# CompVis/stable-diffusion

Measured on NVIDIA B200. Metric: images_per_sec_sdv1_512x512_plms50_cfg7.5, higher is better.
Workload: dtype fp16

## Files before the change

### stable-diffusion_b200/csrc/attention_tc.cu

```cuda
#include "../../include/sdb200.h"
#include "host.h"
#include "ptx.cuh"

#include <stdlib.h>

namespace sdb {

constexpr int AQ = 128;
constexpr int AKV = 64;
template <int DPAD>
struct AttnCfg {
  static constexpr int ST = DPAD <= 128 ? 3 : 2;
  static constexpr int SMEM = AQ * DPAD * 2 + ST * (2 * AKV * DPAD * 2) + 2 * AQ * AKV * 2 + 1024;
};

struct AttnArgs {
  int nq, nkv, d, heads;
  int ldo;
  long long o_batch_stride;
  __half* out;
  float scale_log2;
  int causal;
};

__device__ __forceinline__ float fast_exp2(float x) {
  float y;
  asm("ex2.approx.ftz.f32 %0, %1;" : "=f"(y) : "f"(x));
  return y;
}

template <int DPAD>
__global__ void __launch_bounds__(192)
    attention_tc_kernel(const __grid_constant__ CUtensorMap tmQ, const __grid_constant__ CUtensorMap tmK,
                        const __grid_constant__ CUtensorMap tmV, const AttnArgs p) {
  constexpr int PANELS = DPAD / 64;
  constexpr int Q_BYTES = AQ * DPAD * 2;
  constexpr int K_BYTES = AKV * DPAD * 2;
  constexpr int V_BYTES = DPAD * AKV * 2;
  constexpr int P_BYTES = AQ * AKV * 2;
  constexpr int TMEM_COLS = (128 + DPAD) <= 256 ? 256 : 512;
  constexpr int ST = AttnCfg<DPAD>::ST;
  constexpr uint32_t O_COL = 128;

  extern __shared__ uint8_t smem_raw[];
  uint8_t* smem = smem_raw + ((1024u - (smem_u32(smem_raw) & 1023u)) & 1023u);
  uint8_t* q_s = smem;
  uint8_t* k_s = q_s + Q_BYTES;
  uint8_t* v_s = k_s + ST * K_BYTES;
  uint8_t* p_s = v_s + ST * V_BYTES;

  __shared__ uint64_t q_full, k_full[ST], v_full[ST], kv_empty[ST], s_full[2], p_full[2], pv_done[2];
  __shared__ uint32_t tmem_base_smem;

  const int warp = threadIdx.x >> 5;
  const int lane = threadIdx.x & 31;
  pdl_launch_dependents();
  const int q0 = blockIdx.x * AQ;
  const int head = blockIdx.y;
  const int b = blockIdx.z;
  int nkv_eff = p.nkv;
  if (p.causal) nkv_eff = min(p.nkv, q0 + AQ);
  const int n_iter = (nkv_eff + AKV - 1) / AKV;

  if (warp == 0 && lane == 0) {
    tma_prefetch_desc(&tmQ);
    tma_prefetch_desc(&tmK);
    tma_prefetch_desc(&tmV);
    mbar_init(&q_full, 1);
    for (int i = 0; i < ST; ++i) {
      mbar_init(&k_full[i], 1);
      mbar_init(&v_full[i], 1);
      mbar_init(&kv_empty[i], 1);
    }
    for (int i = 0; i < 2; ++i) {
      mbar_init(&s_full[i], 1);
      mbar_init(&p_full[i], 128);
      mbar_init(&pv_done[i], 1);
    }
    fence_barrier_init();
  }
  if (warp == 1) {
    tmem_alloc(&tmem_base_smem, TMEM_COLS);
    tmem_relinquish();
  }
  tc_fence_before();
  __syncthreads();
  tc_fence_after();
  const uint32_t tmem = tmem_base_smem;

  pdl_wait();
  if (warp == 0) {
    if (elect_one()) {
      mbar_arrive_expect_tx(&q_full, Q_BYTES);
      for (int pn = 0; pn < PANELS; ++pn)
        tma_load_3d(q_s + pn * (AQ * 128), &tmQ, &q_full, head * DPAD + pn * 64, q0, b);
      for (int j = 0; j < n_iter; ++j) {
        int s = j % ST;
        uint32_t ph = (j / ST) & 1;
        mbar_wait(&kv_empty[s], ph ^ 1);
        mbar_arrive_expect_tx(&k_full[s], K_BYTES);
        for (int pn = 0; pn < PANELS; ++pn)
          tma_load_3d(k_s + s * K_BYTES + pn * (AKV * 128), &tmK, &k_full[s], head * DPAD + pn * 64, j * AKV, b);
        mbar_arrive_expect_tx(&v_full[s], V_BYTES);
        tma_load_3d(v_s + s * V_BYTES, &tmV, &v_full[s], j * AKV, head * DPAD, b);
      }
    }
  } else if (warp == 1) {
    if (elect_one()) {
      constexpr uint32_t idesc_s = umma_idesc_f16(AQ, AKV);
      const int ksteps = (p.d + 15) >> 4;
      const uint32_t idesc_o = umma_idesc_f16(AQ, ksteps * 16);
      const uint32_t q_addr = smem_u32(q_s);
      auto issue_s = [&](int j) {
        const int s = j & 1;
        const int ks = j % ST;
        mbar_wait(&k_full[ks], (j / ST) & 1);
        tc_fence_after();
        const uint32_t k_addr = smem_u32(k_s + ks * K_BYTES);
#pragma unroll
        for (int kk = 0; kk < DPAD / 16; ++kk) {
          if (kk >= ksteps) break;
          uint64_t da = umma_desc_k128(q_addr + (kk >> 2) * (AQ * 128) + (kk & 3) * 32);
          uint64_t db = umma_desc_k128(k_addr + (kk >> 2) * (AKV * 128) + (kk & 3) * 32);
          umma_f16(tmem + s * AKV, da, db, idesc_s, kk > 0 ? 1u : 0u);
        }
        umma_commit(&s_full[s]);
      };
      mbar_wait(&q_full, 0);
      if (n_iter > 0) issue_s(0);
      for (int j = 0; j < n_iter; ++j) {
        int s = j & 1;
        uint32_t ph = (j >> 1) & 1;
        if (j + 1 < n_iter) issue_s(j + 1);
        const int ks = j % ST;
        mbar_wait(&p_full[s], ph);
        mbar_wait(&v_full[ks], (j / ST) & 1);
        tc_fence_after();
        const uint32_t p_addr = smem_u32(p_s + s * P_BYTES);
        const uint32_t v_addr = smem_u32(v_s + ks * V_BYTES);
#pragma unroll
        for (int kk = 0; kk < AKV / 16; ++kk) {
          uint64_t da = umma_desc_k128(p_addr + kk * 32);
          uint64_t db = umma_desc_k128(v_addr + kk * 32);
          umma_f16(tmem + O_COL, da, db, idesc_o, (j > 0 || kk > 0) ? 1u : 0u);
        }
        umma_commit(&kv_empty[ks]);
        umma_commit(&pv_done[s]);
      }
    }
  } else {
    const int lg = warp & 3;
    const int r = lg * 32 + lane;
    const int qi = q0 + r;
    const uint32_t lane_addr = static_cast<uint32_t>(lg * 32) << 16;
    float m_used = -INFINITY;
    float l = 0.f;
    for (int j = 0; j < n_iter; ++j) {
      const int s = j & 1;
      mbar_wait(&s_full[s], (j >> 1) & 1);
      tc_fence_after();
      float t[AKV];
      {
        uint32_t r0[32], r1[32];
        tmem_ld32(tmem + lane_addr + s * AKV, r0);
        tmem_ld32(tmem + lane_addr + s * AKV + 32, r1);
        tmem_ld_wait();
#pragma unroll
        for (int c = 0; c < 32; ++c) {
          t[c] = __uint_as_float(r0[c]);
          t[32 + c] = __uint_as_float(r1[c]);
        }
      }
      const int kv0 = j * AKV;
      if ((kv0 + AKV > p.nkv) || (p.causal && kv0 + AKV - 1 > q0)) {
#pragma unroll
        for (int c = 0; c < AKV; ++c) {
          int kv = kv0 + c;
          if ((kv >= p.nkv) || (p.causal && kv > qi)) t[c] = -INFINITY;
        }
      }
      float mx[8];
#pragma unroll
      for (int i = 0; i < 8; ++i) mx[i] = t[i];
#pragma unroll
      for (int c = 8; c < AKV; ++c) mx[c & 7] = fmaxf(mx[c & 7], t[c]);
      const float m_raw = fmaxf(fmaxf(fmaxf(mx[0], mx[1]), fmaxf(mx[2], mx[3])), fmaxf(fmaxf(mx[4], mx[5]), fmaxf(mx[6], mx[7])));
      const float m_blk = m_raw * p.scale_log2;
      if (j == 0) {
        m_used = m_blk;
      } else {
        float m_new = fmaxf(m_used, m_blk);
        bool need = m_new > m_used + 8.0f;
        if (__any_sync(0xffffffffu, need)) {
          mbar_wait(&pv_done[(j - 1) & 1], ((j - 1) >> 1) & 1);
          tc_fence_after();
          float alpha = need ? exp2f(m_used - m_new) : 1.0f;
#pragma unroll 1
          for (int c = 0; c < DPAD / 32; ++c) {
            uint32_t o[32];
            tmem_ld32(tmem + lane_addr + O_COL + c * 32, o);
            tmem_ld_wait();
#pragma unroll
            for (int i = 0; i < 32; ++i) o[i] = __float_as_uint(__uint_as_float(o[i]) * alpha);
            tmem_st32(tmem + lane_addr + O_COL + c * 32, o);
          }
          tmem_st_wait();
          l *= alpha;
          if (need) m_used = m_new;
        }
      }
      float sm[8] = {0.f, 0.f, 0.f, 0.f, 0.f, 0.f, 0.f, 0.f};
      const float neg_m = -m_used;
      if (j >= 2) mbar_wait(&pv_done[s], ((j - 2) >> 1) & 1);
#pragma unroll
      for (int c = 0; c < AKV; ++c) {
        t[c] = fast_exp2(fmaf(t[c], p.scale_log2, neg_m));
        sm[c & 7] += t[c];
      }
      l += ((sm[0] + sm[1]) + (sm[2] + sm[3])) + ((sm[4] + sm[5]) + (sm[6] + sm[7]));
      uint8_t* prow = p_s + s * P_BYTES + r * 128;
#pragma unroll
      for (int c16 = 0; c16 < 8; ++c16) {
        __half2 h0 = __floats2half2_rn(t[c16 * 8 + 0], t[c16 * 8 + 1]);
        __half2 h1 = __floats2half2_rn(t[c16 * 8 + 2], t[c16 * 8 + 3]);
        __half2 h2 = __floats2half2_rn(t[c16 * 8 + 4], t[c16 * 8 + 5]);
        __half2 h3 = __floats2half2_rn(t[c16 * 8 + 6], t[c16 * 8 + 7]);
        uint4 u;
        u.x = *reinterpret_cast<uint32_t*>(&h0);
        u.y = *reinterpret_cast<uint32_t*>(&h1);
        u.z = *reinterpret_cast<uint32_t*>(&h2);
        u.w = *reinterpret_cast<uint32_t*>(&h3);
        *reinterpret_cast<uint4*>(prow + ((c16 ^ (r & 7)) << 4)) = u;
      }
      fence_proxy_async();
      tc_fence_before();
      mbar_arrive(&p_full[s]);
    }
    if (n_iter > 0) {
      mbar_wait(&pv_done[(n_iter - 1) & 1], ((n_iter - 1) >> 1) & 1);
      tc_fence_after();
    }
    const float inv_l = l > 0.f ? 1.0f / l : 0.f;
    __half* orow = p.out + static_cast<size_t>(b) * p.o_batch_stride + static_cast<size_t>(qi) * p.ldo + head * p.d;
#pragma unroll 1
    for (int c = 0; c < DPAD / 32; ++c) {
      if (c * 32 >= p.d) break;
      uint32_t o[32];
      tmem_ld32(tmem + lane_addr + O_COL + c * 32, o);
      tmem_ld_wait();
      if (qi < p.nq && n_iter > 0) {
#pragma unroll
        for (int i = 0; i < 32; i += 2) {
          int col = c * 32 + i;
          if (col < p.d)
            *reinterpret_cast<__half2*>(orow + col) =
                __floats2half2_rn(__uint_as_float(o[i]) * inv_l, __uint_as_float(o[i + 1]) * inv_l);
        }
      }
    }
    tc_fence_before();
  }
  __syncthreads();
  if (warp == 1) {
    tc_fence_after();
    tmem_dealloc(tmem, TMEM_COLS);
  }
}


constexpr int SPLIT_THREADS = 64 + 256;
constexpr int SPLIT_ST = 3;
constexpr int SPLIT_SMEM = AQ * 64 * 2 + SPLIT_ST * (2 * AKV * 64 * 2) + 2 * AQ * AKV * 2 + 1024;

__global__ void __launch_bounds__(SPLIT_THREADS, 2)
    attention_split_kernel(const __grid_constant__ CUtensorMap tmQ, const __grid_constant__ CUtensorMap tmK,
                           const __grid_constant__ CUtensorMap tmV, const AttnArgs p) {
  constexpr int DPAD = 64;
  constexpr int Q_BYTES = AQ * DPAD * 2;
  constexpr int K_BYTES = AKV * DPAD * 2;
  constexpr int V_BYTES = DPAD * AKV * 2;
  constexpr int P_BYTES = AQ * AKV * 2;
  constexpr int TMEM_COLS = 256;
  constexpr int ST = SPLIT_ST;
  constexpr uint32_t O_COL = 128;

  extern __shared__ uint8_t smem_raw[];
  uint8_t* smem = smem_raw + ((1024u - (smem_u32(smem_raw) & 1023u)) & 1023u);
  uint8_t* q_s = smem;
  uint8_t* k_s = q_s + Q_BYTES;
  uint8_t* v_s = k_s + ST * K_BYTES;
  uint8_t* p_s = v_s + ST * V_BYTES;

  __shared__ uint64_t q_full, k_full[ST], v_full[ST], kv_empty[ST], s_full[2], p_full[2], pv_done[2];
  __shared__ uint32_t tmem_base_smem;
  __shared__ float m_sh[2][AQ];

  const int warp = threadIdx.x >> 5;
  const int lane = threadIdx.x & 31;
  pdl_launch_dependents();
  const int q0 = blockIdx.x * AQ;
  const int head = blockIdx.y;
  const int b = blockIdx.z;
  int nkv_eff = p.nkv;
  if (p.causal) nkv_eff = min(p.nkv, q0 + AQ);
  const int n_iter = (nkv_eff + AKV - 1) / AKV;

  if (warp == 0 && lane == 0) {
    tma_prefetch_desc(&tmQ);
    tma_prefetch_desc(&tmK);
    tma_prefetch_desc(&tmV);
    mbar_init(&q_full, 1);
    for (int i = 0; i < ST; ++i) {
      mbar_init(&k_full[i], 1);
      mbar_init(&v_full[i], 1);
      mbar_init(&kv_empty[i], 1);
    }
    for (int i = 0; i < 2; ++i) {
      mbar_init(&s_full[i], 1);
      mbar_init(&p_full[i], 256);
      mbar_init(&pv_done[i], 1);
    }
    fence_barrier_init();
  }
  if (warp == 1) {
    tmem_alloc(&tmem_base_smem, TMEM_COLS);
    tmem_relinquish();
  }
  {
    const int granules = (DPAD - p.d) * 8;
    for (int i = threadIdx.x; i < ST * granules; i += SPLIT_THREADS) {
      const int st = i / granules, g = i - st * granules;
      const uint32_t val = (g < 8) ? 0x3C003C00u : 0u;
      *reinterpret_cast<uint4*>(v_s + st * V_BYTES + p.d * 128 + g * 16) = make_uint4(val, val, val, val);
    }
    fence_proxy_async();
  }
  tc_fence_before();
  __syncthreads();
  tc_fence_after();
  const uint32_t tmem = tmem_base_smem;

  pdl_wait();
  if (warp == 0) {
    if (elect_one()) {
      const uint32_t v_load_bytes = static_cast<uint32_t>(p.d) * AKV * 2;
      mbar_arrive_expect_tx(&q_full, Q_BYTES);
      tma_load_3d(q_s, &tmQ, &q_full, head * DPAD, q0, b);
      for (int j = 0; j < n_iter; ++j) {
        int s = j % ST;
        uint32_t ph = (j / ST) & 1;
        mbar_wait(&kv_empty[s], ph ^ 1);
        mbar_arrive_expect_tx(&k_full[s], K_BYTES);
        tma_load_3d(k_s + s * K_BYTES, &tmK, &k_full[s], head * DPAD, j * AKV, b);
        mbar_arrive_expect_tx(&v_full[s], v_load_bytes);
        tma_load_3d(v_s + s * V_BYTES, &tmV, &v_full[s], j * AKV, head * DPAD, b);
      }
    }
  } else if (warp == 1) {
    if (elect_one()) {
      constexpr uint32_t idesc_s = umma_idesc_f16(AQ, AKV);
      const int ksteps = (p.d + 15) >> 4;
      const uint32_t idesc_o = umma_idesc_f16(AQ, min(DPAD, ((p.d + 16) >> 4) << 4));
      const uint32_t q_addr = smem_u32(q_s);
      auto issue_s = [&](int j) {
        const int s = j & 1;
        const int ks = j % ST;
        mbar_wait(&k_full[ks], (j / ST) & 1);
        tc_fence_after();
        const uint32_t k_addr = smem_u32(k_s + ks * K_BYTES);
#pragma unroll
        for (int kk = 0; kk < DPAD / 16; ++kk) {
          if (kk >= ksteps) break;
          uint64_t da = umma_desc_k128(q_addr + kk * 32);
          uint64_t db = umma_desc_k128(k_addr + kk * 32);
          umma_f16(tmem + s * AKV, da, db, idesc_s, kk > 0 ? 1u : 0u);
        }
        umma_commit(&s_full[s]);
      };
      mbar_wait(&q_full, 0);
      if (n_iter > 0) issue_s(0);
      for (int j = 0; j < n_iter; ++j) {
        int s = j & 1;
        uint32_t ph = (j >> 1) & 1;
        if (j + 1 < n_iter) issue_s(j + 1);
        const int ks = j % ST;
        mbar_wait(&p_full[s], ph);
        mbar_wait(&v_full[ks], (j / ST) & 1);
        tc_fence_after();
        const uint32_t p_addr = smem_u32(p_s + s * P_BYTES);
        const uint32_t v_addr = smem_u32(v_s + ks * V_BYTES);
#pragma unroll
        for (int kk = 0; kk < AKV / 16; ++kk) {
          uint64_t da = umma_desc_k128(p_addr + kk * 32);
          uint64_t db = umma_desc_k128(v_addr + kk * 32);
          umma_f16(tmem + O_COL + (kk >> 1) * DPAD, da, db, idesc_o, (j > 0 || (kk & 1)) ? 1u : 0u);
        }
        umma_commit(&kv_empty[ks]);
        umma_commit(&pv_done[s]);
      }
    }
  } else {
    const int lg = warp & 3;
    const int hf = (warp - 2) >> 2;
    const int r = lg * 32 + lane;
    const int qi = q0 + r;
    const uint32_t lane_addr = static_cast<uint32_t>(lg * 32) << 16;
    const uint32_t o_addr = tmem + lane_addr + O_COL + hf * DPAD;
    float m_used = -INFINITY;
    for (int j = 0; j < n_iter; ++j) {
      const int s = j & 1;
      mbar_wait(&s_full[s], (j >> 1) & 1);
      tc_fence_after();
      float t[32];
      {
        uint32_t r0[32];
        tmem_ld32(tmem + lane_addr + s * AKV + hf * 32, r0);
        tmem_ld_wait();
#pragma unroll
        for (int c = 0; c < 32; ++c) t[c] = __uint_as_float(r0[c]);
      }
      const int kv0 = j * AKV + hf * 32;
      if ((kv0 + 32 > p.nkv) || (p.causal && kv0 + 31 > q0)) {
#pragma unroll
        for (int c = 0; c < 32; ++c) {
          int kv = kv0 + c;
          if ((kv >= p.nkv) || (p.causal && kv > qi)) t[c] = -INFINITY;
        }
      }
      float mx[4];
#pragma unroll
      for (int i = 0; i < 4; ++i) mx[i] = fmaxf(fmaxf(t[i], t[4 + i]), t[8 + i]);
#pragma unroll
      for (int i = 0; i < 4; ++i) mx[i] = fmaxf(fmaxf(mx[i], t[12 + i]), t[16 + i]);
#pragma unroll
      for (int i = 0; i < 4; ++i) mx[i] = fmaxf(fmaxf(mx[i], t[20 + i]), t[24 + i]);
#pragma unroll
      for (int i = 0; i < 4; ++i) mx[i] = fmaxf(mx[i], t[28 + i]);
      const float m_blk = fmaxf(fmaxf(mx[0], mx[1]), fmaxf(mx[2], mx[3])) * p.scale_log2;
      {
        const float m_new = fmaxf(m_used, m_blk);
        const bool need = m_new > m_used + 8.0f;
        if (j > 0 && __any_sync(0xffffffffu, need)) {
          mbar_wait(&pv_done[(j - 1) & 1], ((j - 1) >> 1) & 1);
          tc_fence_after();
          const float alpha = need ? exp2f(m_used - m_new) : 1.0f;
#pragma unroll 1
          for (int c = 0; c < DPAD / 32; ++c) {
            uint32_t o[32];
            tmem_ld32(o_addr + c * 32, o);
            tmem_ld_wait();
#pragma unroll
            for (int i = 0; i < 32; ++i) o[i] = __float_as_uint(__uint_as_float(o[i]) * alpha);
            tmem_st32(o_addr + c * 32, o);
          }
          tmem_st_wait();
        }
        if (need) m_used = m_new;
      }
      const float neg_m = (m_used == -INFINITY) ? 0.f : -m_used;
      if (j >= 2) mbar_wait(&pv_done[s], ((j - 2) >> 1) & 1);
#pragma unroll
      for (int c = 0; c < 32; ++c) t[c] = fast_exp2(fmaf(t[c], p.scale_log2, neg_m));
      uint8_t* prow = p_s + s * P_BYTES + r * 128;
#pragma unroll
      for (int i = 0; i < 4; ++i) {
        __half2 h0 = __floats2half2_rn(t[i * 8 + 0], t[i * 8 + 1]);
        __half2 h1 = __floats2half2_rn(t[i * 8 + 2], t[i * 8 + 3]);
        __half2 h2 = __floats2half2_rn(t[i * 8 + 4], t[i * 8 + 5]);
        __half2 h3 = __floats2half2_rn(t[i * 8 + 6], t[i * 8 + 7]);
        uint4 u;
        u.x = *reinterpret_cast<uint32_t*>(&h0);
        u.y = *reinterpret_cast<uint32_t*>(&h1);
        u.z = *reinterpret_cast<uint32_t*>(&h2);
        u.w = *reinterpret_cast<uint32_t*>(&h3);
        *reinterpret_cast<uint4*>(prow + (((hf * 4 + i) ^ (r & 7)) << 4)) = u;
      }
      fence_proxy_async();
      tc_fence_before();
      mbar_arrive(&p_full[s]);
    }
    m_sh[hf][r] = m_used;
    asm volatile("bar.sync 1, 256;" ::: "memory");
    if (n_iter > 0) {
      mbar_wait(&pv_done[(n_iter - 1) & 1], ((n_iter - 1) >> 1) & 1);
      tc_fence_after();
    }
    const float mA = m_sh[0][r], mB = m_sh[1][r];
    const float m = fmaxf(mA, mB);
    const float fA = (mA == -INFINITY) ? 0.f : exp2f(mA - m);
    const float fB = (mB == -INFINITY) ? 0.f : exp2f(mB - m);
    const uint32_t oa = tmem + lane_addr + O_COL, ob = oa + DPAD;
    float inv_l = 0.f;
    uint32_t a[32], bb[32];
    if (n_iter > 0) {
      const uint32_t la = tmem_ld1(oa + p.d), lb = tmem_ld1(ob + p.d);
      tmem_ld32(oa + hf * 32, a);
      tmem_ld32(ob + hf * 32, bb);
      tmem_ld_wait();
      const float l = fA * __uint_as_float(la) + fB * __uint_as_float(lb);
      inv_l = l > 0.f ? 1.0f / l : 0.f;
    }
    if (qi < p.nq && n_iter > 0) {
      __half* orow = p.out + static_cast<size_t>(b) * p.o_batch_stride + static_cast<size_t>(qi) * p.ldo + head * p.d;
      const float ga = fA * inv_l, gb = fB * inv_l;
#pragma unroll
      for (int i = 0; i < 32; i += 2) {
        const int col = hf * 32 + i;
        if (col < p.d)
          *reinterpret_cast<__half2*>(orow + col) =
              __floats2half2_rn(__uint_as_float(a[i]) * ga + __uint_as_float(bb[i]) * gb,
                                __uint_as_float(a[i + 1]) * ga + __uint_as_float(bb[i + 1]) * gb);
      }
    }
    tc_fence_before();
  }
  __syncthreads();
  if (warp == 1) {
    tc_fence_after();
    tmem_dealloc(tmem, TMEM_COLS);
  }
}


constexpr int WIDE_D = 512;
constexpr int WIDE_DV = 256;
constexpr int WIDE_KST = 4;
constexpr int WIDE_PANELS = WIDE_D / 64;
constexpr int WIDE_SMEM = AQ * WIDE_D * 2 + WIDE_KST * (AKV * 64 * 2) + WIDE_DV * AKV * 2 + AQ * AKV * 2 + 1024;

__global__ void __launch_bounds__(192, 1)
    attention_wide_kernel(const __grid_constant__ CUtensorMap tmQ, const __grid_constant__ CUtensorMap tmK,
                          const __grid_constant__ CUtensorMap tmV, const AttnArgs p) {
  constexpr int Q_BYTES = AQ * WIDE_D * 2;
  constexpr int KP_BYTES = AKV * 64 * 2;
  constexpr int V_BYTES = WIDE_DV * AKV * 2;
  constexpr int TMEM_COLS = 512;
  constexpr uint32_t O_COL = 128;

  extern __shared__ uint8_t smem_raw[];
  uint8_t* smem = smem_raw + ((1024u - (smem_u32(smem_raw) & 1023u)) & 1023u);
  uint8_t* q_s = smem;
  uint8_t* k_s = q_s + Q_BYTES;
  uint8_t* v_s = k_s + WIDE_KST * KP_BYTES;
  uint8_t* p_s = v_s + V_BYTES;

  __shared__ uint64_t q_full, k_full[WIDE_KST], k_empty[WIDE_KST], v_full, s_full[2], p_full, pv_done;
  __shared__ uint32_t tmem_base_smem;

  const int warp = threadIdx.x >> 5;
  const int lane = threadIdx.x & 31;
  pdl_launch_dependents();
  const int q0 = blockIdx.x * AQ;
  const int dv0 = blockIdx.y * WIDE_DV;
  const int b = blockIdx.z;
  const int n_iter = (p.nkv + AKV - 1) / AKV;

  if (warp == 0 && lane == 0) {
    tma_prefetch_desc(&tmQ);
    tma_prefetch_desc(&tmK);
    tma_prefetch_desc(&tmV);
    mbar_init(&q_full, 1);
    for (int i = 0; i < WIDE_KST; ++i) {
      mbar_init(&k_full[i], 1);
      mbar_init(&k_empty[i], 1);
    }
    mbar_init(&v_full, 1);
    mbar_init(&s_full[0], 1);
    mbar_init(&s_full[1], 1);
    mbar_init(&p_full, 128);
    mbar_init(&pv_done, 1);
    fence_barrier_init();
  }
  if (warp == 1) {
    tmem_alloc(&tmem_base_smem, TMEM_COLS);
    tmem_relinquish();
  }
  tc_fence_before();
  __syncthreads();
  tc_fence_after();
  const uint32_t tmem = tmem_base_smem;

  pdl_wait();
  if (warp == 0) {
    if (elect_one()) {
      mbar_arrive_expect_tx(&q_full, Q_BYTES);
      for (int pn = 0; pn < WIDE_PANELS; ++pn) tma_load_3d(q_s + pn * (AQ * 128), &tmQ, &q_full, pn * 64, q0, b);
      int ks = 0;
      uint32_t kph = 0;
      for (int j = 0; j < n_iter; ++j) {
        for (int pn = 0; pn < WIDE_PANELS; ++pn) {
          mbar_wait(&k_empty[ks], kph ^ 1);
          mbar_arrive_expect_tx(&k_full[ks], KP_BYTES);
          tma_load_3d(k_s + ks * KP_BYTES, &tmK, &k_full[ks], pn * 64, j * AKV, b);
          if (++ks == WIDE_KST) {
            ks = 0;
            kph ^= 1;
          }
        }
        if (j > 0) mbar_wait(&pv_done, (j - 1) & 1);
        mbar_arrive_expect_tx(&v_full, V_BYTES);
        tma_load_3d(v_s, &tmV, &v_full, j * AKV, dv0, b);
      }
    }
  } else if (warp == 1) {
    if (elect_one()) {
      constexpr uint32_t idesc_s = umma_idesc_f16(AQ, AKV);
      constexpr uint32_t idesc_o = umma_idesc_f16(AQ, WIDE_DV);
      const uint32_t q_addr = smem_u32(q_s);
      int ks = 0;
      uint32_t kph = 0;
      auto issue_s = [&](int j) {
        const int s = j & 1;
        for (int pn = 0; pn < WIDE_PANELS; ++pn) {
          mbar_wait(&k_full[ks], kph);
          tc_fence_after();
          const uint32_t k_addr = smem_u32(k_s + ks * KP_BYTES);
#pragma unroll
          for (int kk = 0; kk < 4; ++kk) {
            uint64_t da = umma_desc_k128(q_addr + pn * (AQ * 128) + kk * 32);
            uint64_t db = umma_desc_k128(k_addr + kk * 32);
            umma_f16(tmem + s * AKV, da, db, idesc_s, (pn > 0 || kk > 0) ? 1u : 0u);
          }
          umma_commit(&k_empty[ks]);
          if (++ks == WIDE_KST) {
            ks = 0;
            kph ^= 1;
          }
        }
        umma_commit(&s_full[s]);
      };
      mbar_wait(&q_full, 0);
      if (n_iter > 0) issue_s(0);
      for (int j = 0; j < n_iter; ++j) {
        if (j + 1 < n_iter) issue_s(j + 1);
        mbar_wait(&p_full, j & 1);
        mbar_wait(&v_full, j & 1);
        tc_fence_after();
        const uint32_t p_addr = smem_u32(p_s);
        const uint32_t v_addr = smem_u32(v_s);
#pragma unroll
        for (int kk = 0; kk < AKV / 16; ++kk) {
          uint64_t da = umma_desc_k128(p_addr + kk * 32);
          uint64_t db = umma_desc_k128(v_addr + kk * 32);
          umma_f16(tmem + O_COL, da, db, idesc_o, (j > 0 || kk > 0) ? 1u : 0u);
        }
        umma_commit(&pv_done);
      }
    }
  } else {
    const int lg = warp & 3;
    const int r = lg * 32 + lane;
    const int qi = q0 + r;
    const uint32_t lane_addr = static_cast<uint32_t>(lg * 32) << 16;
    float m_used = -INFINITY;
    float l = 0.f;
    for (int j = 0; j < n_iter; ++j) {
      const int s = j & 1;
      mbar_wait(&s_full[s], (j >> 1) & 1);
      tc_fence_after();
      float t[AKV];
      {
        uint32_t r0[32], r1[32];
        tmem_ld32(tmem + lane_addr + s * AKV, r0);
        tmem_ld32(tmem + lane_addr + s * AKV + 32, r1);
        tmem_ld_wait();
#pragma unroll
        for (int c = 0; c < 32; ++c) {
          t[c] = __uint_as_float(r0[c]);
          t[32 + c] = __uint_as_float(r1[c]);
        }
      }
      const int kv0 = j * AKV;
      if (kv0 + AKV > p.nkv) {
#pragma unroll
        for (int c = 0; c < AKV; ++c)
          if (kv0 + c >= p.nkv) t[c] = -INFINITY;
      }
      float mx[8];
#pragma unroll
      for (int i = 0; i < 8; ++i) mx[i] = t[i];
#pragma unroll
      for (int c = 8; c < AKV; ++c) mx[c & 7] = fmaxf(mx[c & 7], t[c]);
      const float m_blk =
          fmaxf(fmaxf(fmaxf(mx[0], mx[1]), fmaxf(mx[2], mx[3])), fmaxf(fmaxf(mx[4], mx[5]), fmaxf(mx[6], mx[7]))) * p.scale_log2;
      if (j == 0) {
        m_used = m_blk;
      } else {
        mbar_wait(&pv_done, (j - 1) & 1);
        tc_fence_after();
        const float m_new = fmaxf(m_used, m_blk);
        const bool need = m_new > m_used + 8.0f;
        if (__any_sync(0xffffffffu, need)) {
          const float alpha = need ? exp2f(m_used - m_new) : 1.0f;
#pragma unroll 1
          for (int c = 0; c < WIDE_DV / 32; ++c) {
            uint32_t o[32];
            tmem_ld32(tmem + lane_addr + O_COL + c * 32, o);
            tmem_ld_wait();
#pragma unroll
            for (int i = 0; i < 32; ++i) o[i] = __float_as_uint(__uint_as_float(o[i]) * alpha);
            tmem_st32(tmem + lane_addr + O_COL + c * 32, o);
          }
          tmem_st_wait();
          l *= alpha;
          if (need) m_used = m_new;
        }
      }
      float sm[8] = {0.f, 0.f, 0.f, 0.f, 0.f, 0.f, 0.f, 0.f};
      const float neg_m = -m_used;
#pragma unroll
      for (int c = 0; c < AKV; ++c) {
        t[c] = fast_exp2(fmaf(t[c], p.scale_log2, neg_m));
        sm[c & 7] += t[c];
      }
      l += ((sm[0] + sm[1]) + (sm[2] + sm[3])) + ((sm[4] + sm[5]) + (sm[6] + sm[7]));
      uint8_t* prow = p_s + r * 128;
#pragma unroll
      for (int c16 = 0; c16 < 8; ++c16) {
        __half2 h0 = __floats2half2_rn(t[c16 * 8 + 0], t[c16 * 8 + 1]);
        __half2 h1 = __floats2half2_rn(t[c16 * 8 + 2], t[c16 * 8 + 3]);
        __half2 h2 = __floats2half2_rn(t[c16 * 8 + 4], t[c16 * 8 + 5]);
        __half2 h3 = __floats2half2_rn(t[c16 * 8 + 6], t[c16 * 8 + 7]);
        uint4 u;
        u.x = *reinterpret_cast<uint32_t*>(&h0);
        u.y = *reinterpret_cast<uint32_t*>(&h1);
        u.z = *reinterpret_cast<uint32_t*>(&h2);
        u.w = *reinterpret_cast<uint32_t*>(&h3);
        *reinterpret_cast<uint4*>(prow + ((c16 ^ (r & 7)) << 4)) = u;
      }
      fence_proxy_async();
      tc_fence_before();
      mbar_arrive(&p_full);
    }
    if (n_iter > 0) {
      mbar_wait(&pv_done, (n_iter - 1) & 1);
      tc_fence_after();
    }
    const float inv_l = l > 0.f ? 1.0f / l : 0.f;
    __half* orow = p.out + static_cast<size_t>(b) * p.o_batch_stride + static_cast<size_t>(qi) * p.ldo + dv0;
#pragma unroll 1
    for (int c = 0; c < WIDE_DV / 32; ++c) {
      uint32_t o[32];
      tmem_ld32(tmem + lane_addr + O_COL + c * 32, o);
      tmem_ld_wait();
      if (qi < p.nq && n_iter > 0) {
#pragma unroll
        for (int i = 0; i < 32; i += 8) {
          __half2 h0 = __floats2half2_rn(__uint_as_float(o[i]) * inv_l, __uint_as_float(o[i + 1]) * inv_l);
          __half2 h1 = __floats2half2_rn(__uint_as_float(o[i + 2]) * inv_l, __uint_as_float(o[i + 3]) * inv_l);
          __half2 h2 = __floats2half2_rn(__uint_as_float(o[i + 4]) * inv_l, __uint_as_float(o[i + 5]) * inv_l);
          __half2 h3 = __floats2half2_rn(__uint_as_float(o[i + 6]) * inv_l, __uint_as_float(o[i + 7]) * inv_l);
          uint4 u;
          u.x = *reinterpret_cast<uint32_t*>(&h0);
          u.y = *reinterpret_cast<uint32_t*>(&h1);
          u.z = *reinterpret_cast<uint32_t*>(&h2);
          u.w = *reinterpret_cast<uint32_t*>(&h3);
          *reinterpret_cast<uint4*>(orow + c * 32 + i) = u;
        }
      }
    }
    tc_fence_before();
  }
  __syncthreads();
  if (warp == 1) {
    tc_fence_after();
    tmem_dealloc(tmem, TMEM_COLS);
  }
}

template <int DPAD>
static int launch_attn(const CUtensorMap& q, const CUtensorMap& k, const CUtensorMap& v, const AttnArgs& p, dim3 grid,
                       cudaStream_t st) {
  constexpr int SMEM = AttnCfg<DPAD>::SMEM;
  auto kern = attention_tc_kernel<DPAD>;
  static bool configured = false;
  if (!configured) {
    SDB_CUDA(cudaFuncSetAttribute(kern, cudaFuncAttributeMaxDynamicSharedMemorySize, SMEM));
    configured = true;
  }
  SDB_CUDA(launch_pdl(kern, grid, dim3(192), SMEM, st, q, k, v, p));
  SDB_LAUNCH_CHECK();
  return 0;
}

}

using namespace sdb;
// ... 108 lines not shown
```

### stable-diffusion_b200/csrc/ptx.cuh

```cuda
#pragma once
#include <cuda.h>
#include <cuda_fp16.h>
#include <cuda_runtime.h>
#include <stdint.h>
#include <stdio.h>

namespace sdb {

__device__ __forceinline__ uint32_t smem_u32(const void* p) {
  return static_cast<uint32_t>(__cvta_generic_to_shared(p));
}

__device__ __forceinline__ bool elect_one() {
  uint32_t pred;
  asm volatile(
      "{\n\t.reg .pred P;\n\t"
      "elect.sync _|P, 0xffffffff;\n\t"
      "selp.u32 %0, 1, 0, P;\n\t}\n"
      : "=r"(pred));
  return pred != 0;
}

__device__ __forceinline__ void pdl_launch_dependents() { asm volatile("griddepcontrol.launch_dependents;" ::: "memory"); }
__device__ __forceinline__ void pdl_wait() { asm volatile("griddepcontrol.wait;" ::: "memory"); }

__device__ __forceinline__ uint32_t cluster_ctarank() {
  uint32_t r;
  asm volatile("mov.u32 %0, %%cluster_ctarank;" : "=r"(r));
  return r;
}
__device__ __forceinline__ uint32_t cluster_id_x() {
  uint32_t r;
  asm volatile("mov.u32 %0, %%clusterid.x;" : "=r"(r));
  return r;
}
__device__ __forceinline__ uint32_t cluster_nctaid_x() {
  uint32_t r;
  asm volatile("mov.u32 %0, %%nclusterid.x;" : "=r"(r));
  return r;
}
__device__ __forceinline__ uint32_t mapa_shared(uint32_t smem_addr, uint32_t rank) {
  uint32_t r;
  asm volatile("mapa.shared::cluster.u32 %0, %1, %2;" : "=r"(r) : "r"(smem_addr), "r"(rank));
  return r;
}
__device__ __forceinline__ void cluster_arrive() { asm volatile("barrier.cluster.arrive.release.aligned;" ::: "memory"); }
__device__ __forceinline__ void cluster_wait() { asm volatile("barrier.cluster.wait.acquire.aligned;" ::: "memory"); }
__device__ __forceinline__ void cluster_sync_all() {
  cluster_arrive();
  cluster_wait();
}
__device__ __forceinline__ void st_cluster_f32x4(uint32_t addr, float a, float b, float c, float d) {
  asm volatile("st.shared::cluster.v4.f32 [%0], {%1, %2, %3, %4};" ::"r"(addr), "f"(a), "f"(b), "f"(c), "f"(d) : "memory");
}

__device__ __forceinline__ void mbar_init(uint64_t* bar, uint32_t count) {
  asm volatile("mbarrier.init.shared::cta.b64 [%0], %1;" ::"r"(smem_u32(bar)), "r"(count) : "memory");
}
__device__ __forceinline__ void fence_barrier_init() {
  asm volatile("fence.mbarrier_init.release.cluster;" ::: "memory");
}
__device__ __forceinline__ void fence_proxy_async() {
  asm volatile("fence.proxy.async.shared::cta;" ::: "memory");
}
__device__ __forceinline__ void mbar_arrive_expect_tx(uint64_t* bar, uint32_t bytes) {
  asm volatile("mbarrier.arrive.expect_tx.shared::cta.b64 _, [%0], %1;" ::"r"(smem_u32(bar)), "r"(bytes)
               : "memory");
}
__device__ __forceinline__ void mbar_arrive(uint64_t* bar) {
  asm volatile("mbarrier.arrive.shared::cta.b64 _, [%0];" ::"r"(smem_u32(bar)) : "memory");
}
__device__ __forceinline__ void mbar_arrive_cluster(uint32_t cluster_addr) {
  asm volatile("mbarrier.arrive.release.cluster.shared::cluster.b64 _, [%0];" ::"r"(cluster_addr) : "memory");
}
__device__ __forceinline__ void mbar_arrive_expect_tx_cluster(uint32_t cluster_addr, uint32_t bytes) {
  asm volatile("mbarrier.arrive.expect_tx.release.cluster.shared::cluster.b64 _, [%0], %1;" ::"r"(cluster_addr), "r"(bytes)
               : "memory");
}
__device__ __forceinline__ bool mbar_try_wait(uint64_t* bar, uint32_t parity) {
  uint32_t ok;
  asm volatile(
      "{\n\t.reg .pred p;\n\t"
      "mbarrier.try_wait.parity.shared::cta.b64 p, [%1], %2, %3;\n\t"
      "selp.u32 %0, 1, 0, p;\n\t}\n"
      : "=r"(ok)
      : "r"(smem_u32(bar)), "r"(parity), "r"(2000u)
      : "memory");
  return ok != 0;
}
static __device__ __noinline__ void mbar_timeout(uint32_t bar_addr, uint32_t parity) {
  printf("sdb: mbarrier wait timeout block(%d,%d,%d) thread %d bar@%u parity %u\n", blockIdx.x, blockIdx.y, blockIdx.z,
         threadIdx.x, bar_addr, parity);
  __trap();
}
__device__ __forceinline__ void mbar_wait(uint64_t* bar, uint32_t parity) {
  uint32_t spins = 0;
  while (!mbar_try_wait(bar, parity)) {
    if (++spins == (1u << 24)) mbar_timeout(smem_u32(bar), parity);
  }
}

__device__ __forceinline__ void tma_prefetch_desc(const CUtensorMap* m) {
  asm volatile("prefetch.tensormap [%0];" ::"l"(reinterpret_cast<uint64_t>(m)) : "memory");
}
__device__ __forceinline__ void tma_load_2d(void* smem, const CUtensorMap* m, uint64_t* bar, int c0, int c1) {
  asm volatile(
      "cp.async.bulk.tensor.2d.shared::cluster.global.mbarrier::complete_tx::bytes [%0], [%1, {%3, %4}], [%2];" ::"r"(
          smem_u32(smem)),
      "l"(reinterpret_cast<uint64_t>(m)), "r"(smem_u32(bar)), "r"(c0), "r"(c1)
      : "memory");
}
__device__ __forceinline__ void tma_load_3d(void* smem, const CUtensorMap* m, uint64_t* bar, int c0, int c1, int c2) {
  asm volatile(
      "cp.async.bulk.tensor.3d.shared::cluster.global.mbarrier::complete_tx::bytes [%0], [%1, {%3, %4, %5}], [%2];" ::
          "r"(smem_u32(smem)),
      "l"(reinterpret_cast<uint64_t>(m)), "r"(smem_u32(bar)), "r"(c0), "r"(c1), "r"(c2)
      : "memory");
}
__device__ __forceinline__ void tma_load_4d(void* smem, const CUtensorMap* m, uint64_t* bar, int c0, int c1, int c2,
                                            int c3) {
  asm volatile(
      "cp.async.bulk.tensor.4d.shared::cluster.global.mbarrier::complete_tx::bytes [%0], [%1, {%3, %4, %5, %6}], "
      "[%2];" ::"r"(smem_u32(smem)),
      "l"(reinterpret_cast<uint64_t>(m)), "r"(smem_u32(bar)), "r"(c0), "r"(c1), "r"(c2), "r"(c3)
      : "memory");
}

__device__ __forceinline__ void tma_load_2d_cg2(void* smem, const CUtensorMap* m, uint32_t bar_cluster_addr, int c0, int c1) {
  asm volatile(
      "cp.async.bulk.tensor.2d.cta_group::2.shared::cluster.global.mbarrier::complete_tx::bytes [%0], [%1, {%3, %4}], [%2];" ::
          "r"(smem_u32(smem)),
      "l"(reinterpret_cast<uint64_t>(m)), "r"(bar_cluster_addr), "r"(c0), "r"(c1)
      : "memory");
}
__device__ __forceinline__ void tma_load_4d_cg2(void* smem, const CUtensorMap* m, uint32_t bar_cluster_addr, int c0, int c1,
                                                int c2, int c3) {
  asm volatile(
      "cp.async.bulk.tensor.4d.cta_group::2.shared::cluster.global.mbarrier::complete_tx::bytes [%0], [%1, {%3, %4, %5, %6}], "
      "[%2];" ::"r"(smem_u32(smem)),
      "l"(reinterpret_cast<uint64_t>(m)), "r"(bar_cluster_addr), "r"(c0), "r"(c1), "r"(c2), "r"(c3)
      : "memory");
}

__device__ __forceinline__ void tma_load_2d_addr(uint32_t dst, const CUtensorMap* m, uint32_t bar, int c0, int c1) {
  asm volatile(
      "cp.async.bulk.tensor.2d.shared::cluster.global.mbarrier::complete_tx::bytes [%0], [%1, {%3, %4}], [%2];" ::"r"(dst),
      "l"(reinterpret_cast<uint64_t>(m)), "r"(bar), "r"(c0), "r"(c1)
      : "memory");
}
__device__ __forceinline__ void tma_load_4d_addr(uint32_t dst, const CUtensorMap* m, uint32_t bar, int c0, int c1, int c2,
                                                 int c3) {
  asm volatile(
      "cp.async.bulk.tensor.4d.shared::cluster.global.mbarrier::complete_tx::bytes [%0], [%1, {%3, %4, %5, %6}], "
      "[%2];" ::"r"(dst),
      "l"(reinterpret_cast<uint64_t>(m)), "r"(bar), "r"(c0), "r"(c1), "r"(c2), "r"(c3)
      : "memory");
}
__device__ __forceinline__ void tma_load_2d_cg2_addr(uint32_t dst, const CUtensorMap* m, uint32_t bar, int c0, int c1) {
  asm volatile(
      "cp.async.bulk.tensor.2d.cta_group::2.shared::cluster.global.mbarrier::complete_tx::bytes [%0], [%1, {%3, %4}], [%2];" ::
          "r"(dst),
      "l"(reinterpret_cast<uint64_t>(m)), "r"(bar), "r"(c0), "r"(c1)
      : "memory");
}
__device__ __forceinline__ void tma_load_4d_cg2_addr(uint32_t dst, const CUtensorMap* m, uint32_t bar, int c0, int c1,
                                                     int c2, int c3) {
  asm volatile(
      "cp.async.bulk.tensor.4d.cta_group::2.shared::cluster.global.mbarrier::complete_tx::bytes [%0], [%1, {%3, %4, %5, %6}], "
      "[%2];" ::"r"(dst),
      "l"(reinterpret_cast<uint64_t>(m)), "r"(bar), "r"(c0), "r"(c1), "r"(c2), "r"(c3)
      : "memory");
}

__device__ __forceinline__ void tma_load_5d(void* smem, const CUtensorMap* m, uint64_t* bar, int c0, int c1, int c2, int c3,
                                            int c4) {
  asm volatile(
      "cp.async.bulk.tensor.5d.shared::cluster.global.mbarrier::complete_tx::bytes [%0], [%1, {%3, %4, %5, %6, %7}], "
      "[%2];" ::"r"(smem_u32(smem)),
      "l"(reinterpret_cast<uint64_t>(m)), "r"(smem_u32(bar)), "r"(c0), "r"(c1), "r"(c2), "r"(c3), "r"(c4)
      : "memory");
}

__device__ __forceinline__ void tma_store_5d(const CUtensorMap* m, const void* smem, int c0, int c1, int c2, int c3,
                                             int c4) {
  asm volatile(
      "cp.async.bulk.tensor.5d.global.shared::cta.bulk_group [%0, {%2, %3, %4, %5, %6}], [%1];" ::"l"(
          reinterpret_cast<uint64_t>(m)),
      "r"(smem_u32(smem)), "r"(c0), "r"(c1), "r"(c2), "r"(c3), "r"(c4)
      : "memory");
}
__device__ __forceinline__ void tma_store_commit() { asm volatile("cp.async.bulk.commit_group;" ::: "memory"); }
template <int N>
__device__ __forceinline__ void tma_store_wait_read() {
  asm volatile("cp.async.bulk.wait_group.read %0;" ::"n"(N) : "memory");
}
template <int N>
__device__ __forceinline__ void tma_store_wait() {
  asm volatile("cp.async.bulk.wait_group %0;" ::"n"(N) : "memory");
}

__device__ __forceinline__ void tmem_alloc(uint32_t* dst_smem, uint32_t ncols) {
  asm volatile("tcgen05.alloc.cta_group::1.sync.aligned.shared::cta.b32 [%0], %1;" ::"r"(smem_u32(dst_smem)),
               "r"(ncols)
               : "memory");
}
__device__ __forceinline__ void tmem_relinquish() {
  asm volatile("tcgen05.relinquish_alloc_permit.cta_group::1.sync.aligned;" ::: "memory");
}
__device__ __forceinline__ void tmem_dealloc(uint32_t taddr, uint32_t ncols) {
  asm volatile("tcgen05.dealloc.cta_group::1.sync.aligned.b32 %0, %1;" ::"r"(taddr), "r"(ncols) : "memory");
}
__device__ __forceinline__ void tmem_alloc_cg2(uint32_t* dst_smem, uint32_t ncols) {
  asm volatile("tcgen05.alloc.cta_group::2.sync.aligned.shared::cta.b32 [%0], %1;" ::"r"(smem_u32(dst_smem)),
               "r"(ncols)
               : "memory");
}
__device__ __forceinline__ void tmem_relinquish_cg2() {
  asm volatile("tcgen05.relinquish_alloc_permit.cta_group::2.sync.aligned;" ::: "memory");
}
__device__ __forceinline__ void tmem_dealloc_cg2(uint32_t taddr, uint32_t ncols) {
  asm volatile("tcgen05.dealloc.cta_group::2.sync.aligned.b32 %0, %1;" ::"r"(taddr), "r"(ncols) : "memory");
}
__device__ __forceinline__ void tc_fence_before() { asm volatile("tcgen05.fence::before_thread_sync;" ::: "memory"); }
__device__ __forceinline__ void tc_fence_after() { asm volatile("tcgen05.fence::after_thread_sync;" ::: "memory"); }

__device__ __forceinline__ void umma_f16(uint32_t tmem_d, uint64_t desc_a, uint64_t desc_b, uint32_t idesc,
                                         uint32_t accumulate) {
  asm volatile(
      "{\n\t.reg .pred p;\n\t"
      "setp.ne.b32 p, %4, 0;\n\t"
      "tcgen05.mma.cta_group::1.kind::f16 [%0], %1, %2, %3, p;\n\t}\n" ::"r"(tmem_d),
      "l"(desc_a), "l"(desc_b), "r"(idesc), "r"(accumulate)
      : "memory");
}
__device__ __forceinline__ void umma_f16_w(uint32_t tmem_d, uint32_t a_lo, uint32_t b_lo, uint32_t desc_hi, uint32_t idesc,
                                           uint32_t accumulate) {
  asm volatile(
      "{\n\t.reg .pred p;\n\t.reg .b64 da, db;\n\t"
      "mov.b64 da, {%1, %3};\n\t"
      "mov.b64 db, {%2, %3};\n\t"
      "setp.ne.b32 p, %5, 0;\n\t"
      "tcgen05.mma.cta_group::1.kind::f16 [%0], da, db, %4, p;\n\t}\n" ::"r"(tmem_d),
      "r"(a_lo), "r"(b_lo), "r"(desc_hi), "r"(idesc), "r"(accumulate)
      : "memory");
}
__device__ __forceinline__ void umma_f16_cg2_w(uint32_t tmem_d, uint32_t a_lo, uint32_t b_lo, uint32_t desc_hi,
                                               uint32_t idesc, uint32_t accumulate) {
  asm volatile(
      "{\n\t.reg .pred p;\n\t.reg .b64 da, db;\n\t"
      "mov.b64 da, {%1, %3};\n\t"
      "mov.b64 db, {%2, %3};\n\t"
      "setp.ne.b32 p, %5, 0;\n\t"
      "tcgen05.mma.cta_group::2.kind::f16 [%0], da, db, %4, p;\n\t}\n" ::"r"(tmem_d),
      "r"(a_lo), "r"(b_lo), "r"(desc_hi), "r"(idesc), "r"(accumulate)
      : "memory");
}
__device__ __forceinline__ void umma_commit(uint64_t* bar) {
  asm volatile("tcgen05.commit.cta_group::1.mbarrier::arrive::one.shared::cluster.b64 [%0];" ::"r"(smem_u32(bar))
               : "memory");
}

__device__ __forceinline__ void umma_f16_cg2(uint32_t tmem_d, uint64_t desc_a, uint64_t desc_b, uint32_t idesc,
                                             uint32_t accumulate) {
  asm volatile(
      "{\n\t.reg .pred p;\n\t"
      "setp.ne.b32 p, %4, 0;\n\t"
      "tcgen05.mma.cta_group::2.kind::f16 [%0], %1, %2, %3, p;\n\t}\n" ::"r"(tmem_d),
      "l"(desc_a), "l"(desc_b), "r"(idesc), "r"(accumulate)
      : "memory");
}
__device__ __forceinline__ void umma_commit_cg2(uint64_t* bar, uint16_t cta_mask) {
  asm volatile("tcgen05.commit.cta_group::2.mbarrier::arrive::one.shared::cluster.multicast::cluster.b64 [%0], %1;" ::"r"(
                   smem_u32(bar)),
               "h"(cta_mask)
               : "memory");
}

__device__ __forceinline__ uint64_t umma_desc_k128(uint32_t smem_addr) {
  uint64_t d = 0;
  d |= static_cast<uint64_t>((smem_addr & 0x3FFFF) >> 4);
  d |= static_cast<uint64_t>(1024 >> 4) << 32;
  d |= static_cast<uint64_t>(1) << 46;
  d |= static_cast<uint64_t>(2) << 61;
  return d;
}
__host__ __device__ constexpr uint32_t umma_idesc_f16(int M, int N) {
  return (1u << 4) | (0u << 7) | (0u << 10) | (0u << 15) | (0u << 16) | (static_cast<uint32_t>(N >> 3) << 17) |
         (static_cast<uint32_t>(M >> 4) << 24);
}

__device__ __forceinline__ void tmem_ld32(uint32_t taddr, uint32_t (&r)[32]) {
  asm volatile(
      "tcgen05.ld.sync.aligned.32x32b.x32.b32 "
      "{%0, %1, %2, %3, %4, %5, %6, %7, %8, %9, %10, %11, %12, %13, %14, %15, "
      "%16, %17, %18, %19, %20, %21, %22, %23, %24, %25, %26, %27, %28, %29, %30, %31}, [%32];"
      : "=r"(r[0]), "=r"(r[1]), "=r"(r[2]), "=r"(r[3]), "=r"(r[4]), "=r"(r[5]), "=r"(r[6]), "=r"(r[7]), "=r"(r[8]),
        "=r"(r[9]), "=r"(r[10]), "=r"(r[11]), "=r"(r[12]), "=r"(r[13]), "=r"(r[14]), "=r"(r[15]), "=r"(r[16]),
        "=r"(r[17]), "=r"(r[18]), "=r"(r[19]), "=r"(r[20]), "=r"(r[21]), "=r"(r[22]), "=r"(r[23]), "=r"(r[24]),
        "=r"(r[25]), "=r"(r[26]), "=r"(r[27]), "=r"(r[28]), "=r"(r[29]), "=r"(r[30]), "=r"(r[31])
      : "r"(taddr)
      : "memory");
}
__device__ __forceinline__ uint32_t tmem_ld1(uint32_t taddr) {
  uint32_t r;
  asm volatile("tcgen05.ld.sync.aligned.32x32b.x1.b32 {%0}, [%1];" : "=r"(r) : "r"(taddr) : "memory");
  return r;
}
__device__ __forceinline__ void tmem_ld_wait() { asm volatile("tcgen05.wait::ld.sync.aligned;" ::: "memory"); }
__device__ __forceinline__ void tmem_st32(uint32_t taddr, const uint32_t (&r)[32]) {
  asm volatile(
      "tcgen05.st.sync.aligned.32x32b.x32.b32 [%0], "
      "{%1, %2, %3, %4, %5, %6, %7, %8, %9, %10, %11, %12, %13, %14, %15, %16, "
      "%17, %18, %19, %20, %21, %22, %23, %24, %25, %26, %27, %28, %29, %30, %31, %32};" ::"r"(taddr),
      "r"(r[0]), "r"(r[1]), "r"(r[2]), "r"(r[3]), "r"(r[4]), "r"(r[5]), "r"(r[6]), "r"(r[7]), "r"(r[8]), "r"(r[9]),
      "r"(r[10]), "r"(r[11]), "r"(r[12]), "r"(r[13]), "r"(r[14]), "r"(r[15]), "r"(r[16]), "r"(r[17]), "r"(r[18]),
      "r"(r[19]), "r"(r[20]), "r"(r[21]), "r"(r[22]), "r"(r[23]), "r"(r[24]), "r"(r[25]), "r"(r[26]), "r"(r[27]),
      "r"(r[28]), "r"(r[29]), "r"(r[30]), "r"(r[31])
      : "memory");
}
__device__ __forceinline__ void tmem_st_wait() { asm volatile("tcgen05.wait::st.sync.aligned;" ::: "memory"); }

__device__ __forceinline__ uint32_t sw128_offset(int row, int col, int rows) {
  int panel = col >> 6;
  int c16 = (col & 63) >> 3;
  return static_cast<uint32_t>(panel * rows * 128 + row * 128 + ((c16 ^ (row & 7)) << 4) + ((col & 7) << 1));
}

}
```

Before: 4.209.

## Keep softmax probabilities in TMEM and schedule per-half S/PV MMAs independently

The split attention kernel no longer writes P to shared memory. It packs the fp16 probabilities back into TMEM over the S accumulator and runs the PV MMA with A taken from TMEM. The S and PV work is also split per 32-column half, each with its own barriers, and the MMA warp polls them non-blockingly so each half can move ahead on its own. This removes the shared-memory P buffer, its stores and the proxy fence, and lowers smem use. The cost is a more complex polling scheduler with nanosleep. Correctness depends on the TMEM-A operand layout and the aliasing of S and P in the same TMEM columns.

```diff
diff --git a/stable-diffusion_b200/csrc/attention_tc.cu b/stable-diffusion_b200/csrc/attention_tc.cu
--- a/stable-diffusion_b200/csrc/attention_tc.cu
+++ b/stable-diffusion_b200/csrc/attention_tc.cu
@@ -270,7 +270,7 @@
 
 constexpr int SPLIT_THREADS = 64 + 256;
 constexpr int SPLIT_ST = 3;
-constexpr int SPLIT_SMEM = AQ * 64 * 2 + SPLIT_ST * (2 * AKV * 64 * 2) + 2 * AQ * AKV * 2 + 1024;
+constexpr int SPLIT_SMEM = AQ * 64 * 2 + SPLIT_ST * (2 * AKV * 64 * 2) + 1024;
 
 __global__ void __launch_bounds__(SPLIT_THREADS, 2)
     attention_split_kernel(const __grid_constant__ CUtensorMap tmQ, const __grid_constant__ CUtensorMap tmK,
@@ -279,7 +279,6 @@
   constexpr int Q_BYTES = AQ * DPAD * 2;
   constexpr int K_BYTES = AKV * DPAD * 2;
   constexpr int V_BYTES = DPAD * AKV * 2;
-  constexpr int P_BYTES = AQ * AKV * 2;
   constexpr int TMEM_COLS = 256;
   constexpr int ST = SPLIT_ST;
   constexpr uint32_t O_COL = 128;
@@ -289,9 +288,8 @@
   uint8_t* q_s = smem;
   uint8_t* k_s = q_s + Q_BYTES;
   uint8_t* v_s = k_s + ST * K_BYTES;
-  uint8_t* p_s = v_s + ST * V_BYTES;
-
-  __shared__ uint64_t q_full, k_full[ST], v_full[ST], kv_empty[ST], s_full[2], p_full[2], pv_done[2];
+
+  __shared__ uint64_t q_full, k_full[ST], v_full[ST], kv_empty[ST], s_full[2][2], p_full[2][2], pv_done[2][2];
   __shared__ uint32_t tmem_base_smem;
   __shared__ float m_sh[2][AQ];
 
@@ -313,13 +311,14 @@
     for (int i = 0; i < ST; ++i) {
       mbar_init(&k_full[i], 1);
       mbar_init(&v_full[i], 1);
-      mbar_init(&kv_empty[i], 1);
-    }
-    for (int i = 0; i < 2; ++i) {
-      mbar_init(&s_full[i], 1);
-      mbar_init(&p_full[i], 256);
-      mbar_init(&pv_done[i], 1);
-    }
+      mbar_init(&kv_empty[i], 2);
+    }
+    for (int h = 0; h < 2; ++h)
+      for (int i = 0; i < 2; ++i) {
+        mbar_init(&s_full[h][i], 1);
+        mbar_init(&p_full[h][i], 128);
+        mbar_init(&pv_done[h][i], 1);
+      }
     fence_barrier_init();
   }
   if (warp == 1) {
@@ -358,45 +357,55 @@
     }
   } else if (warp == 1) {
     if (elect_one()) {
-      constexpr uint32_t idesc_s = umma_idesc_f16(AQ, AKV);
+      constexpr uint32_t idesc_s = umma_idesc_f16(AQ, 32);
       const int ksteps = (p.d + 15) >> 4;
       const uint32_t idesc_o = umma_idesc_f16(AQ, min(DPAD, ((p.d + 16) >> 4) << 4));
       const uint32_t q_addr = smem_u32(q_s);
-      auto issue_s = [&](int j) {
-        const int s = j & 1;
-        const int ks = j % ST;
-        mbar_wait(&k_full[ks], (j / ST) & 1);
-        tc_fence_after();
-        const uint32_t k_addr = smem_u32(k_s + ks * K_BYTES);
-#pragma unroll
-        for (int kk = 0; kk < DPAD / 16; ++kk) {
-          if (kk >= ksteps) break;
-          uint64_t da = umma_desc_k128(q_addr + kk * 32);
-          uint64_t db = umma_desc_k128(k_addr + kk * 32);
-          umma_f16(tmem + s * AKV, da, db, idesc_s, kk > 0 ? 1u : 0u);
-        }
-        umma_commit(&s_full[s]);
-      };
       mbar_wait(&q_full, 0);
-      if (n_iter > 0) issue_s(0);
-      for (int j = 0; j < n_iter; ++j) {
-        int s = j & 1;
-        uint32_t ph = (j >> 1) & 1;
-        if (j + 1 < n_iter) issue_s(j + 1);
-        const int ks = j % ST;
-        mbar_wait(&p_full[s], ph);
-        mbar_wait(&v_full[ks], (j / ST) & 1);
-        tc_fence_after();
-        const uint32_t p_addr = smem_u32(p_s + s * P_BYTES);
-        const uint32_t v_addr = smem_u32(v_s + ks * V_BYTES);
-#pragma unroll
-        for (int kk = 0; kk < AKV / 16; ++kk) {
-          uint64_t da = umma_desc_k128(p_addr + kk * 32);
-          uint64_t db = umma_desc_k128(v_addr + kk * 32);
-          umma_f16(tmem + O_COL + (kk >> 1) * DPAD, da, db, idesc_o, (j > 0 || (kk & 1)) ? 1u : 0u);
-        }
-        umma_commit(&kv_empty[ks]);
-        umma_commit(&pv_done[s]);
+      int s_next[2] = {0, 0}, pv_next[2] = {0, 0};
+      uint32_t idle = 0;
+      while (pv_next[0] < n_iter || pv_next[1] < n_iter) {
+        bool progress = false;
+#pragma unroll
+        for (int h = 0; h < 2; ++h) {
+          const int jp = pv_next[h];
+          if (jp < s_next[h] && mbar_test_wait(&p_full[h][jp & 1], (jp >> 1) & 1) &&
+              mbar_test_wait(&v_full[jp % ST], (jp / ST) & 1)) {
+            tc_fence_after();
+            const uint32_t v_addr = smem_u32(v_s + (jp % ST) * V_BYTES) + h * 64;
+#pragma unroll
+            for (int k2 = 0; k2 < 2; ++k2) {
+              uint64_t db = umma_desc_k128(v_addr + k2 * 32);
+              umma_f16_tmem_a(tmem + O_COL + h * DPAD, tmem + (jp & 1) * AKV + h * 32 + k2 * 8, db, idesc_o,
+                              (jp > 0 || k2) ? 1u : 0u);
+            }
+            umma_commit(&kv_empty[jp % ST]);
+            umma_commit(&pv_done[h][jp & 1]);
+            pv_next[h] = jp + 1;
+            progress = true;
+          }
+          const int js = s_next[h];
+          if (js < n_iter && js <= pv_next[h] + 1 && mbar_test_wait(&k_full[js % ST], (js / ST) & 1)) {
+            tc_fence_after();
+            const uint32_t k_addr = smem_u32(k_s + (js % ST) * K_BYTES) + h * 32 * 128;
+#pragma unroll
+            for (int kk = 0; kk < DPAD / 16; ++kk) {
+              if (kk >= ksteps) break;
+              uint64_t da = umma_desc_k128(q_addr + kk * 32);
+              uint64_t db = umma_desc_k128(k_addr + kk * 32);
+              umma_f16(tmem + (js & 1) * AKV + h * 32, da, db, idesc_s, kk > 0 ? 1u : 0u);
+            }
+            umma_commit(&s_full[h][js & 1]);
+            s_next[h] = js + 1;
+            progress = true;
+          }
+        }
+        if (progress) {
+          idle = 0;
+        } else {
+          if (++idle == (1u << 24)) mbar_timeout(smem_u32(&p_full[0][0]), pv_next[0] * 2 + pv_next[1]);
+          __nanosleep(32);
+        }
       }
     }
   } else {
@@ -409,7 +418,7 @@
     float m_used = -INFINITY;
     for (int j = 0; j < n_iter; ++j) {
       const int s = j & 1;
-      mbar_wait(&s_full[s], (j >> 1) & 1);
+      mbar_wait(&s_full[hf][s], (j >> 1) & 1);
       tc_fence_after();
       float t[32];
       {
@@ -441,7 +450,7 @@
         const float m_new = fmaxf(m_used, m_blk);
         const bool need = m_new > m_used + 8.0f;
         if (j > 0 && __any_sync(0xffffffffu, need)) {
-          mbar_wait(&pv_done[(j - 1) & 1], ((j - 1) >> 1) & 1);
+          mbar_wait(&pv_done[hf][(j - 1) & 1], ((j - 1) >> 1) & 1);
           tc_fence_after();
           const float alpha = need ? exp2f(m_used - m_new) : 1.0f;
 #pragma unroll 1
@@ -458,31 +467,24 @@
         if (need) m_used = m_new;
       }
       const float neg_m = (m_used == -INFINITY) ? 0.f : -m_used;
-      if (j >= 2) mbar_wait(&pv_done[s], ((j - 2) >> 1) & 1);
 #pragma unroll
       for (int c = 0; c < 32; ++c) t[c] = fast_exp2(fmaf(t[c], p.scale_log2, neg_m));
-      uint8_t* prow = p_s + s * P_BYTES + r * 128;
-#pragma unroll
-      for (int i = 0; i < 4; ++i) {
-        __half2 h0 = __floats2half2_rn(t[i * 8 + 0], t[i * 8 + 1]);
-        __half2 h1 = __floats2half2_rn(t[i * 8 + 2], t[i * 8 + 3]);
-        __half2 h2 = __floats2half2_rn(t[i * 8 + 4], t[i * 8 + 5]);
-        __half2 h3 = __floats2half2_rn(t[i * 8 + 6], t[i * 8 + 7]);
-        uint4 u;
-        u.x = *reinterpret_cast<uint32_t*>(&h0);
-        u.y = *reinterpret_cast<uint32_t*>(&h1);
-        u.z = *reinterpret_cast<uint32_t*>(&h2);
-        u.w = *reinterpret_cast<uint32_t*>(&h3);
-        *reinterpret_cast<uint4*>(prow + (((hf * 4 + i) ^ (r & 7)) << 4)) = u;
-      }
-      fence_proxy_async();
+      uint32_t pk[16];
+#pragma unroll
+      for (int i = 0; i < 16; ++i) {
+        __half2 h = __floats2half2_rn(t[2 * i], t[2 * i + 1]);
+        pk[i] = *reinterpret_cast<uint32_t*>(&h);
+      }
+      tmem_st16(tmem + lane_addr + s * AKV + hf * 32, pk);
+      tmem_st_wait();
       tc_fence_before();
-      mbar_arrive(&p_full[s]);
+      mbar_arrive(&p_full[hf][s]);
     }
     m_sh[hf][r] = m_used;
     asm volatile("bar.sync 1, 256;" ::: "memory");
     if (n_iter > 0) {
-      mbar_wait(&pv_done[(n_iter - 1) & 1], ((n_iter - 1) >> 1) & 1);
+      mbar_wait(&pv_done[0][(n_iter - 1) & 1], ((n_iter - 1) >> 1) & 1);
+      mbar_wait(&pv_done[1][(n_iter - 1) & 1], ((n_iter - 1) >> 1) & 1);
       tc_fence_after();
     }
     const float mA = m_sh[0][r], mB = m_sh[1][r];
diff --git a/stable-diffusion_b200/csrc/ptx.cuh b/stable-diffusion_b200/csrc/ptx.cuh
--- a/stable-diffusion_b200/csrc/ptx.cuh
+++ b/stable-diffusion_b200/csrc/ptx.cuh
@@ -88,6 +88,17 @@
       : "memory");
   return ok != 0;
 }
+__device__ __forceinline__ bool mbar_test_wait(uint64_t* bar, uint32_t parity) {
+  uint32_t ok;
+  asm volatile(
+      "{\n\t.reg .pred p;\n\t"
+      "mbarrier.test_wait.parity.shared::cta.b64 p, [%1], %2;\n\t"
+      "selp.u32 %0, 1, 0, p;\n\t}\n"
+      : "=r"(ok)
+      : "r"(smem_u32(bar)), "r"(parity)
+      : "memory");
+  return ok != 0;
+}
 static __device__ __noinline__ void mbar_timeout(uint32_t bar_addr, uint32_t parity) {
   printf("sdb: mbarrier wait timeout block(%d,%d,%d) thread %d bar@%u parity %u\n", blockIdx.x, blockIdx.y, blockIdx.z,
          threadIdx.x, bar_addr, parity);
@@ -231,6 +242,15 @@
       "setp.ne.b32 p, %4, 0;\n\t"
       "tcgen05.mma.cta_group::1.kind::f16 [%0], %1, %2, %3, p;\n\t}\n" ::"r"(tmem_d),
       "l"(desc_a), "l"(desc_b), "r"(idesc), "r"(accumulate)
+      : "memory");
+}
+__device__ __forceinline__ void umma_f16_tmem_a(uint32_t tmem_d, uint32_t tmem_a, uint64_t desc_b, uint32_t idesc,
+                                                uint32_t accumulate) {
+  asm volatile(
+      "{\n\t.reg .pred p;\n\t"
+      "setp.ne.b32 p, %4, 0;\n\t"
+      "tcgen05.mma.cta_group::1.kind::f16 [%0], [%1], %2, %3, p;\n\t}\n" ::"r"(tmem_d),
+      "r"(tmem_a), "l"(desc_b), "r"(idesc), "r"(accumulate)
       : "memory");
 }
 __device__ __forceinline__ void umma_f16_w(uint32_t tmem_d, uint32_t a_lo, uint32_t b_lo, uint32_t desc_hi, uint32_t idesc,
@@ -318,6 +338,14 @@
       "r"(r[28]), "r"(r[29]), "r"(r[30]), "r"(r[31])
       : "memory");
 }
+__device__ __forceinline__ void tmem_st16(uint32_t taddr, const uint32_t (&r)[16]) {
+  asm volatile(
+      "tcgen05.st.sync.aligned.32x32b.x16.b32 [%0], "
+      "{%1, %2, %3, %4, %5, %6, %7, %8, %9, %10, %11, %12, %13, %14, %15, %16};" ::"r"(taddr),
+      "r"(r[0]), "r"(r[1]), "r"(r[2]), "r"(r[3]), "r"(r[4]), "r"(r[5]), "r"(r[6]), "r"(r[7]), "r"(r[8]), "r"(r[9]),
+      "r"(r[10]), "r"(r[11]), "r"(r[12]), "r"(r[13]), "r"(r[14]), "r"(r[15])
+      : "memory");
+}
 __device__ __forceinline__ void tmem_st_wait() { asm volatile("tcgen05.wait::st.sync.aligned;" ::: "memory"); }
 
 __device__ __forceinline__ uint32_t sw128_offset(int row, int col, int rows) {
```

Result: faster. 4.270 (median of 6 runs) (+1.4%).
